# angela000/DQNFlappyBird

Hardware: AMD Instinct MI355X
Metric: env steps/sec (whole node) + DQN grad-steps/sec, 80x80x4 batch=32 (higher is better)
Workload: dtype f32

## Files before the change

dqnflappybird_amd/_lib.py:

```python
import ctypes as C
import os

_HERE = os.path.dirname(os.path.abspath(__file__))
LIB_PATH = os.environ.get("FB_LIB") or os.path.join(_HERE, "libfbdqn.so")
ASSET_BLOB = os.path.join(_HERE, "assets", "sprites.bin")

FB_OK = 0
REPLAY_UNIFORM, REPLAY_PER = 0, 1
RNG_CPYTHON, RNG_PHILOX, RNG_NUMPY = 0, 1, 2
ARCH_PLAIN, ARCH_DUELING, ARCH_C51, ARCH_C51_DUELING = 0, 1, 2, 3
NET_ONLINE, NET_TARGET = 0, 1
ALGO_DQN, ALGO_NATURE, ALGO_DOUBLE, ALGO_PER, ALGO_PG = 0, 1, 2, 3, 4
ALGO_C51, ALGO_C51_DOUBLE = 5, 6
ALGO_C51_PER, ALGO_C51_DOUBLE_PER = 7, 8
C51_MAX_ATOMS = 64
ARCH_QR, ARCH_QR_DUELING = 4, 5
ALGO_QR, ALGO_QR_DOUBLE, ALGO_QR_PER, ALGO_QR_DOUBLE_PER = 9, 10, 11, 12
ALGO_MDQN, ALGO_MDQN_PER = 14, 15
MDQN_DEFAULTS = (0.03, 0.9, -1.0)
ALGO_DOUBLE_PER = 16
ARCH_AC = 6
AC_DEFAULTS = (0.5, 0.01)
ARCH_SAC = 7
SAC_DEFAULTS = (0.2, 0.98, 0.0)
# ... 109 lines not shown
    "fb_qnet_set_iqn_risk": [_vp, _f],
    "fb_qnet_get_iqn": [_vp, _vp, _vp, _vp, _vp, _vp],
    "fb_qnet_set_iqn_munchausen": [_vp, _i, _f, _f, _f],
    "fb_qnet_get_iqn_munchausen": [_vp, _vp, _vp, _vp, _vp],
    "fb_qnet_forward_iqn": [_vp, _i, _vp, _i, _vp, _i, _vp, _vp],
    "fb_iqn_draw_taus": [_i, _i, _u64, _u64, _i, _vp, _vp],
    "fb_qnet_iqn_train_step": [_vp, _i, _i, _vp, _vp, _vp, _vp, _vp, _vp, _vp, _u64, _u64, _d, _vp, _vp, _vp, _vp],
    "fb_iqn_train_from_replay": [_vp, _vp, _i, _i, _vp, _vp, _vp, _vp, _vp, _vp, _u64, _u64, _d, _vp, _vp, _vp, _vp],
    "fb_iqn_step": [_vp, _vp, _vp, _vp, _i, _i, _i, _f, _u64, _u64, _i, _d, _vp],
    "fb_qnet_iqn_per_train_step": [_vp, _i, _i, _vp, _vp, _vp, _vp, _vp, _vp, _vp, _vp, _u64, _u64, _d, _vp, _vp, _vp, _vp, _vp],
    "fb_iqn_per_train_from_replay": [_vp, _vp, _i, _i, _vp, _vp, _vp, _vp, _vp, _vp, _vp, _u64, _u64, _d, _vp, _vp, _vp, _vp, _vp],
    "fb_iqn_per_step": [_vp, _vp, _vp, _vp, _i, _i, _i, _f, _u64, _u64, _i, _d, _vp],
    "fb_qnet_destroy": [_vp],
    "fb_qnet_num_params": [_vp, _vp],
    "fb_qnet_init_params": [_vp, _i, _u64, _vp],
    "fb_qnet_load_params": [_vp, _i, _vp, _vp],
    "fb_qnet_store_params": [_vp, _i, _vp, _vp],
    "fb_qnet_get_adam_state": [_vp] * 4,
    "fb_qnet_set_adam_state": [_vp] * 4,
    "fb_qnet_set_hparams": [_vp, _f, _f, _f, _f],
    "fb_qnet_set_inference_dtype": [_vp, _i],
    "fb_qnet_overflow_count": [_vp, _i, _vp],
    "fb_qnet_split_stats": [_vp, _vp, _vp],
    "fb_vec_step_set_schedule": [_i],
    "fb_qnet_set_train_dtype": [_vp, _i],
    "fb_qnet_forward": [_vp, _i, _vp, _i, _vp, _vp],
    "fb_qnet_act": [_vp, _vp, _i, _f, _u64, _u64, _vp, _vp, _vp],
    "fb_qnet_act_nib": [_vp, _vp, _i, _f, _u64, _u64, _vp, _vp, _vp],
    "fb_qnet_train_step": [_vp, _i, _i] + [_vp] * 6 + [_d] + [_vp] * 5,
    "fb_qnet_apply_adam": [_vp, _vp, _vp],
    "fb_train_steps": [_vp, _vp, _i, _i, _i] + [_vp] * 7 + [_d, _vp],
    "fb_qnet_sync_target": [_vp, _vp],
    "fb_qnet_profile_kernel": [_vp, _i, _i, _i, _i] + [_vp] * 7,
    "fb_dist_probe": [C.c_char_p],
    "fb_dist_unique_id": [C.c_char_p, _vp],
    "fb_dist_create": [C.c_char_p, _i, _i, _vp],
    "fb_dist_destroy": [_vp],
    "fb_dist_set_overlap": [_vp, _i],
    "fb_vec_step_dp": [_vp, _vp, _vp, _vp, _vp, _i, _i, _i, _f, _u64, _u64, _i, _d, _i, _vp],
    "fb_dist_reduce_apply": [_vp, _vp, _vp, _i, _vp],
    "fb_dist_grad_event": [_vp],
    "fb_dist_all_reduce": [_vp, _vp, _i64, _vp],
    "fb_qnet_set_grad_event": [_vp, _vp],
    "fb_qnet_grad_split": [_vp],
    "fb_train_from_replay": [_vp, _vp, _i, _i, _vp, _vp, _vp, _vp, _vp, _d, _vp, _vp, _vp, _vp],
    "fb_profile_ring_kernel": [_vp, _vp, _i, _i, _i, _i] + [_vp] * 6,
    "fb_qnet_kernel_name": [_i],
    "fb_vec_step": [_vp, _vp, _vp, _vp, _i, _i, _i, _f, _u64, _u64, _i, _d, _vp],
    "fb_eval_create": [_i, _vp, _sz, _vp],
    "fb_eval_destroy": [_vp],
    "fb_eval_run": [_vp, _vp, _i, _i, _i64, _f, _u64, _u64, _vp, _vp, _vp, _vp, _vp],
    "fb_eval_stats": [_vp, _vp, _vp],
    "fb_eval_q": [_vp, _vp, _i, _vp, _vp],
}


class StepBuffers(C.Structure):
    _fields_ = [(n, C.c_void_p) for n in ("nib", "actions", "frame_bits", "reward", "terminal", "score", "idx", "s", "s2", "a", "t",
                                           "r", "loss", "flat_grad", "isw", "isw32", "abs_err")]


class AcRolloutBuffers(C.Structure):
    _fields_ = [(n, C.c_void_p) for n in ("nib", "actions", "frame_bits", "reward", "terminal", "score", "value", "logp")] + [("slots", C.c_int)]


_lib = None
# ... 55 lines not shown
```

dqnflappybird_amd/csrc/fb_qnet.hip:

```cpp
#include <math.h>
#include <stdlib.h>
#include "fb_common.h"

#ifndef FK_ABL
#define FK_ABL 0
#endif
#ifndef BW_ABL
#define BW_ABL 0
#endif

namespace {

typedef float f32x16 __attribute__((ext_vector_type(16)));

constexpr int OFF_W1 = 0, OFF_B1 = 8192, OFF_W2 = 8224, OFF_B2 = 40992, OFF_W3 = 41056, OFF_B3 = 77920,
              OFF_WF1 = 77984;
constexpr int CONV_PARAMS = OFF_WF1;
#include "fb_head.h"
#include "fb_sampler.h"
#include "fb_gather.h"
constexpr int MAXTB = 256;


struct Slice { const float *params; const uint8_t *states; int s_off, count; const uint16_t *w1s; int fshift; };
// ... 1831 lines not shown
    if (threadIdx.x >= 256) return;
    const int reg = threadIdx.x >> 6, row = 4 * g + reg, col = r, mr = m0 + row, unit = n0 + col;
    float v = red[reg * 64 + lane];
#pragma unroll
    for (int w = 1; w < 8; w++) v += red[(w * 4 + reg) * 64 + lane];
    const bool live = mr < M;
    const size_t srow = (size_t)s.s_off + (live ? mr : M - 1);
    if (live) a.hf[srow * a.FC + unit] = v;
    if (!a.qpart || FK_ABL == 4) return;
    const float h = fmaxf(v + hb, 0.f);
    const int qs = a.A + 1;
    float *qo = a.qpart + (srow * (size_t)gridDim.y + blockIdx.y) * qs;
#pragma unroll
    for (int c = 0; c <= MAXA; c++) {
        if (c < a.A || (c == a.A && a.dueling)) {
            float x = h * (c == a.A ? hw[MAXA] : hw[c]);
#pragma unroll
            for (int o = 8; o > 0; o >>= 1) x += __shfl_xor(x, o, 16);
            if (col == 0 && live) qo[c] = x;
        }
    }
}

struct Bw1Args {
    int algo, B, FC, A, dueling, stot, n_dx, rb;
    NetOff off;
    const float *params, *pnext, *ptarget;
    const float *hf, *qpart, *h3;
    const uint8_t *act; const float *rew; const uint8_t *term; const float *isw;
    double gamma;
    float *grad, *dh3, *loss, *abs_err, *y_out;
    AdamDev *adam; int tick;
    FbGate gate;
};
constexpr int BW_DX_ROW = 4;
constexpr int BW_DW_ROW = 36;

template <int AT, bool DX, bool MD = false, bool DP = false, bool HU = false>
__device__ __forceinline__ void fc1_bwd2_body(const Bw1Args &L, float *smem, const MdPar M = MdPar{}, const float delta = 0.f) {
    const int tid = threadIdx.x, lane = tid & 63, wave = tid >> 6, B = L.B, FC = L.FC, A = AT == MAXA ? L.A : AT;
    const float *P = L.params;
    float (*dadv)[MAXA] = reinterpret_cast<float (*)[MAXA]>(smem);
    float *dv = smem + MAXTB * MAXA, *lterm = dv + MAXTB, *dadv2 = lterm + MAXTB, *big = dadv2 + 2 * MAXTB;
    const bool lead = blockIdx.x == 0;
    const bool dbl = DP || L.algo == FB_ALGO_DOUBLE;
    const bool row3 = MD || dbl;
    const int qs = A + 1, ntile = FC >> 4;
    constexpr bool dx_role = DX;
    const int mt = dx_role ? blockIdx.x / 50 : 0, t2 = dx_role ? 0 : blockIdx.x - L.n_dx, nt = t2 / 7, kg = t2 - nt * 7;
    const int kt = dx_role ? blockIdx.x - mt * 50 : kg * 8 + wave;
    auto unit_params = [&](int n, float &bias, float (&wq)[AT], float &wv) {
        bias = P[L.off.bf1 + n];
        wv = P[(L.dueling ? L.off.wv : L.off.bf1) + n];
#pragma unroll
        for (int c = 0; c < AT; c++) wq[c] = P[L.off.wq + n * A + (c < A ? c : 0)];
    };
    float pre_hf[32], pre_bias, pre_wq[AT], pre_wv, pre_a[16];
    float4 pre_w[8];
    if constexpr (DX) {
        const int ch = FC < 512 ? FC : 512, n = tid < ch ? tid : 0;
#pragma unroll
        for (int q = 0; q < 32; q++) { const int bq_ = mt * 32 + q; pre_hf[q] = L.hf[(size_t)(bq_ < B ? bq_ : 0) * FC + n]; }
        unit_params(n, pre_bias, pre_wq, pre_wv);
        const int kh = ch / 16, nbeg = wave * (ch / 8) + (lane >> 5) * kh;
        const float *brun = P + OFF_WF1 + (size_t)(kt * 32 + (lane & 31)) * FC + nbeg;
#pragma unroll
        for (int q = 0; q < 8; q++) pre_w[q] = *reinterpret_cast<const float4 *>(brun + (4 * q < kh ? 4 * q : 0));
#pragma unroll
        for (int q = 0; q < 16; q++) pre_a[q] = 0.f;
#pragma unroll
        for (int q = 0; q < 2; q++) { const int mr = mt * 32 + drow(2 * (wave & 7) + q, lane); pre_a[q] = L.h3[(size_t)(mr < B ? mr : 0) * 1600 + kt * 32 + (lane & 31)]; }
    } else {
        const int c = tid & 31;
#pragma unroll
        for (int q = 0; q < 2; q++) { const int b = (tid >> 5) + 16 * q; pre_hf[q] = L.hf[(size_t)(b < B ? b : 0) * FC + nt * 32 + c]; }
#pragma unroll
        for (int q = 2; q < 32; q++) pre_hf[q] = 0.f;
        unit_params(nt * 32 + c, pre_bias, pre_wq, pre_wv);
        const int ktc = kt < 50 ? kt : 0;
#pragma unroll
        for (int t = 0; t < 16; t++) { const int b = 2 * t + (lane >> 5); pre_a[t] = L.h3[(size_t)(b < B ? b : 0) * 1600 + ktc * 32 + (lane & 31)]; }
#pragma unroll
        for (int q = 0; q < 8; q++) pre_w[q] = make_float4(0.f, 0.f, 0.f, 0.f);
// ... 172 lines not shown
                }
            }
            __syncthreads();
            const int kh = ch / 16, nbeg = wave * (ch / 8) + hl * kh;
            const float *arun = dh + i * RS + nbeg;
            float4 xa[8];
#pragma unroll
            for (int q = 0; q < 8; q++) xa[q] = *reinterpret_cast<const float4 *>(arun + (4 * q < kh ? 4 * q : 0));
#pragma unroll
            for (int q = 0; q < 8; q++) { keep(xa[q].x); keep(xa[q].y); keep(xa[q].z); keep(xa[q].w); }
#pragma unroll
            for (int q = 0; q < 8; q++) {
                if (4 * q < kh && BW_ABL != 3) {
                    const float4 x = xa[q], w = pre_w[q];
                    const bool rb = L.rb;
                    acc = mfma(rbf(x.x, rb), rbf(w.x, rb), acc); acc = mfma(rbf(x.y, rb), rbf(w.y, rb), acc);
                    acc = mfma(rbf(x.z, rb), rbf(w.z, rb), acc); acc = mfma(rbf(x.w, rb), rbf(w.w, rb), acc);
                }
            }
        }
        reduce_rows<8>(acc, red, wave, lane, mt * 32, B, [&](float v, int r, int mr) {
            const size_t o = (size_t)mr * 1600 + kt * 32 + jj;
            L.dh3[o] = BW_ABL == 4 ? v : (((r & 1) ? pre_a[1] : pre_a[0]) > 0.f ? v : 0.f);
        });
        return;
    }
    if (BW_ABL == 5) return;
    float *dh = big, *hh = big + MAXTB * BW_DW_ROW;
    {
        const int c = tid & 31;
#pragma unroll
        for (int q = 0; q < 2; q++) {
            const int b = (tid >> 5) + 16 * q;
            if (b < B) { float hv; dh[b * BW_DW_ROW + c] = dhf_of(b, pre_hf[q], pre_bias, pre_wq, pre_wv, hv); hh[b * BW_DW_ROW + c] = hv; }
        }
        for (int b = (tid >> 5) + 32; b < B; b += 16) {
            float hv;
            dh[b * BW_DW_ROW + c] = dhf_of(b, L.hf[(size_t)b * FC + nt * 32 + c], pre_bias, pre_wq, pre_wv, hv);
            hh[b * BW_DW_ROW + c] = hv;
        }
    }
    __syncthreads();
    if (kt < 50) {
        f32x16 acc = {0};
#pragma unroll
        for (int t = 0; t < 16; t++) {
            const int b = 2 * t + hl;
            const float w = dh[(b < B ? b : 0) * BW_DW_ROW + jj];
            acc = mfma(b < B ? rbf(pre_a[t], L.rb) : 0.f, b < B ? rbf(w, L.rb) : 0.f, acc);
        }
#pragma unroll 4
        for (int t = 16; t < (B + 1) / 2; t++) {
            const int b = 2 * t + hl, bc = b < B ? b : 0;
            const float x = L.h3[(size_t)bc * 1600 + kt * 32 + i], w = dh[bc * BW_DW_ROW + jj];
            acc = mfma(b < B ? rbf(x, L.rb) : 0.f, b < B ? rbf(w, L.rb) : 0.f, acc);
        }
#pragma unroll
        for (int r = 0; r < 16; r++) L.grad[OFF_WF1 + (size_t)(kt * 32 + drow(r, lane)) * FC + nt * 32 + jj] = acc[r];
    }
    if (kg != 0) return;
    float *part = hh + MAXTB * BW_DW_ROW;
    {
        const int c = tid & 31, pt = tid >> 5;
        float gw[AT], gv = 0.f, gb = 0.f;
#pragma unroll
        for (int q = 0; q < AT; q++) gw[q] = 0.f;
        for (int b = pt; b < B; b += 16) {
            const float h = hh[b * BW_DW_ROW + c];
#pragma unroll
            for (int q = 0; q < AT; q++) if (q < A) gw[q] = fmaf(h, dadv[b][q], gw[q]);
            gv = fmaf(h, dv[b], gv);
            gb += dh[b * BW_DW_ROW + c];
// ... 403 lines not shown
    auto ld = [&](int ks) {
        const int b0 = 16 * (k0 + ks) + 8 * hl;
        float a[8], bb[8];
#pragma unroll
        for (int j = 0; j < 8; j++) {
            const bool ok = b0 + j < B;
            const size_t bc = ok ? b0 + j : 0;
            const float x = pa[bc * 1600], y = pb[bc * FC];
            a[j] = ok ? x : 0.f; bb[j] = ok ? y : 0.f;
        }
        return FragF{make_float4(a[0], a[1], a[2], a[3]), make_float4(a[4], a[5], a[6], a[7]), make_float4(bb[0], bb[1], bb[2], bb[3]),
                     make_float4(bb[4], bb[5], bb[6], bb[7])};
    };
    const Pow2 G = pow2_scale(wave_max(gm));
    if constexpr (KW > 0) {
        FragF f[KW];
#pragma unroll
        for (int q = 0; q < KW; q++) f[q] = ld(q);
#pragma unroll
        for (int q = 0; q < KW; q++) mma_frag<NS, false>(f[q], acc, acl, G.s, bad);
    } else {
        for (int q = 0; q < per; q++) mma_frag<NS, false>(ld(q), acc, acl, G.s, bad);
    }
    if constexpr (NS == 3) {
#pragma unroll
        for (int q = 0; q < 16; q++) acc[q] = fmaf(acl[q], F16_LO_UNSCALE, acc[q]) * G.inv;
        note_overflow(bad, ovf);
    }
    reduce_rows<8>(acc, red, wave, lane, 0, 32, [&](float v, int, int row32) {
        grad[OFF_WF1 + (size_t)(it * 32 + row32) * FC + nt * 32 + r] = v;
    });
}

__device__ __forceinline__ void adam4(float4 &P, float4 &Mv, float4 &V, const float4 Gv, float alpha, float omb1, float omb2, float eps) {
#define FB_ADAM1(c)                                  \
    Mv.c += (Gv.c - Mv.c) * omb1;                    \
    V.c += (Gv.c * Gv.c - V.c) * omb2;               \
    P.c -= (Mv.c * alpha) / (sqrtf(V.c) + eps);
    FB_ADAM1(x) FB_ADAM1(y) FB_ADAM1(z) FB_ADAM1(w)
#undef FB_ADAM1
}

struct AdamSpan { float *p, *m, *v; const float *g; const AdamDev *ad; int q0, q1; };
__device__ __forceinline__ void adam_span_body(int blk, int nblk, const AdamSpan a) {
    const float alpha = a.ad->alpha, omb1 = 1.f - a.ad->b1, omb2 = 1.f - a.ad->b2, eps = a.ad->eps;
    for (int q = a.q0 + blk * (int)blockDim.x + (int)threadIdx.x; q < a.q1; q += nblk * (int)blockDim.x) {
        float4 P = reinterpret_cast<float4 *>(a.p)[q], Mv = reinterpret_cast<float4 *>(a.m)[q], V = reinterpret_cast<float4 *>(a.v)[q];
        adam4(P, Mv, V, reinterpret_cast<const float4 *>(a.g)[q], alpha, omb1, omb2, eps);
        reinterpret_cast<float4 *>(a.p)[q] = P; reinterpret_cast<float4 *>(a.m)[q] = Mv; reinterpret_cast<float4 *>(a.v)[q] = V;
    }
}

constexpr int DW1_IMG_W = 104, DW1_IMG_H = 84, DW1_IMG = DW1_IMG_H * DW1_IMG_W * 4;
constexpr int DW1_STEPS = 30;

template <int NSP> struct Dw1Lds { static constexpr int U4 = DW1_IMG / 16 + (DW1_STEPS / NSP) * 2 * 64 + 64 + 4; };

struct Dw1Ring { const unsigned long long *bits, *fo; };
template <int NSP, bool RING = false>
__device__ __forceinline__ void conv1_dw2_body(int blk, const uint8_t *__restrict__ states, const float *__restrict__ dp1,
                                               const uint8_t *__restrict__ amax, float *__restrict__ slabs, size_t slab_stride, uint4 *pool,
                                               Dw1Ring ring = Dw1Ring{nullptr, nullptr}) {
    constexpr int SW = DW1_STEPS / NSP, PU = (SW + 7) / 8;
    uint4 *img4 = pool, *bfr = pool + DW1_IMG / 16;
    float (*bsum)[32] = reinterpret_cast<float (*)[32]>(bfr + SW * 2 * 64);
    float *sx = reinterpret_cast<float *>(bfr + SW * 2 * 64 + 64);
    const int b = blk / NSP, part = blk - b * NSP, s0 = part * SW;
    const int tid = threadIdx.x, lane = tid & 63, wave = tid >> 6, hl = lane >> 5, c = lane & 31;
    uint8_t *img = reinterpret_cast<uint8_t *>(img4);
    float dv[PU][4];
    int am[PU][4];
#pragma unroll
    for (int u = 0; u < PU; u++) {
        const int ls = wave + 8 * u, g = 2 * (s0 + ls) + hl, oy = g / 3, ox0 = (g - 3 * oy) * 8;
#pragma unroll
        for (int q = 0; q < 4; q++) {
            const int px = (ox0 >> 1) + q;
            const bool ok = ls < SW && px < 10;
            const uint32_t po = ((uint32_t)b * 100u + (uint32_t)(ok ? (oy >> 1) * 10 + px : 0)) * 32u + (uint32_t)c;
            dv[u][q] = dp1[po]; am[u][q] = amax[po];
        }
    }
// ... 281 lines not shown
    Ops cur = fetch(0);
#pragma unroll
    for (int ls = 0; ls < SW; ls++) {
        Ops nxt = cur;
        if (ls + 1 < SW) nxt = fetch(ls + 1);
        uint4 A;
        {
            const f32x2 p0 = {(float)cur.x[0], (float)cur.x[1]}, p1 = {(float)cur.x[2], (float)cur.x[3]};
            const f32x2 p2 = {(float)cur.x[4], (float)cur.x[5]}, p3 = {(float)cur.x[6], (float)cur.x[7]};
            A.x = __builtin_bit_cast(uint32_t, __builtin_convertvector(p0, f16x2)); A.y = __builtin_bit_cast(uint32_t, __builtin_convertvector(p1, f16x2));
            A.z = __builtin_bit_cast(uint32_t, __builtin_convertvector(p2, f16x2)); A.w = __builtin_bit_cast(uint32_t, __builtin_convertvector(p3, f16x2));
        }
        acc = mfma_h(A, cur.bh, acc);
        acl = mfma_h(A, cur.bl, acl);
        cur = nxt;
    }
    float *o = slabs + (size_t)blk * slab_stride;
#pragma unroll
    for (int r = 0; r < 16; r++) o[OFF_W1 + (ky * 32 + drow(r, lane)) * 32 + c] = fmaf(acl[r], F16_LO_UNSCALE, acc[r]) * S1.inv;
    if (wave == 0 && hl == 0) {
        float sum = bsum[0][c];
#pragma unroll
        for (int w = 1; w < 8; w++) sum += bsum[w][c];
        o[OFF_B1 + c] = sum;
    }
}

#ifndef CBW_ABL
#define CBW_ABL 0
#endif
template <int NS, bool RING>
__global__ __launch_bounds__(512) void conv_bw_kernel(BxArgs bx, int B, float *__restrict__ slabs, size_t slab_stride, float *__restrict__ slabs1,
                                                      size_t stride1, const uint8_t *__restrict__ states, const uint8_t *__restrict__ amax, Dw1Ring ring,
                                                      int n_adam, AdamSpan span, FbSampleRider rider, int rb, FbGate gate) {
    __shared__ uint4 pool[BwLds<NS>::U4];
    if (fb_gate_workgroup(gate)) return;
    static_assert(BwLds<NS>::U4 * 16 >= FB_SAMPLE_LDS_WORDS * 4, "the sampler rider borrows the pool");
    uint4 *aux = pool + BwLds<NS>::CH;
    float *dp1s = reinterpret_cast<float *>(aux + BW_AUX_U4);
    const int rid = rider.k ? 1 : 0, bid = (int)blockIdx.x - rid, tid = threadIdx.x;
    if (bid < 0) {
        uint32_t *sw = reinterpret_cast<uint32_t *>(pool);
        if (tid < 64) sample_cpython_body(rider.ctx, rider.k, rider.setsize, rider.out, sw, reinterpret_cast<int *>(sw + 624));
        return;
    }
    if (bid < 2 * B) {
        if (CBW_ABL == 5 || CBW_ABL == 6 || CBW_ABL == 7 || CBW_ABL == 8 || CBW_ABL == 11) return;
        const int b = bid >> 1, part = bid & 1;
        const Bw1Pre pre = bw1_request<RING>(b, part, states, amax, ring);
        for (int i = tid; i < BW1_IMG_U4; i += 512) aux[i] = make_uint4(0u, 0u, 0u, 0u);
        conv32_bx_body<NS, 1>(bx, b, pool, dp1s);
        bw1_put(pre, part, aux);
        __syncthreads();
        if (CBW_ABL == 1 || CBW_ABL == 10) { if (dp1s[tid] == 12345.f) slabs1[0] = 1.f; return; }
        bw1_main(bid, part, pre, dp1s, aux, pool + (BwLds<NS>::CH - 2048 - 4), slabs1, stride1);
        return;
    }
    if (bid < (2 + BW_NW2) * B) {
        if (CBW_ABL == 6 || CBW_ABL == 7 || CBW_ABL == 9 || CBW_ABL == 10) return;
        const int b = (bid - 2 * B) / BW_NW2, sub = (bid - 2 * B) - b * BW_NW2;
        float *p1s = reinterpret_cast<float *>(aux), *dys = p1s + 3200;
        const float4 *src = reinterpret_cast<const float4 *>(bx.p1 + (size_t)b * 3200);
        const float4 xa = src[tid], xb = src[tid < 288 ? 512 + tid : 0];
        reinterpret_cast<float4 *>(p1s)[tid] = xa;
        if (tid < 288) reinterpret_cast<float4 *>(p1s)[512 + tid] = xb;
        conv32_bx_body<NS, 2>(bx, b, pool, dys);
        __syncthreads();
        float *o = slabs + (size_t)b * slab_stride;
        if (CBW_ABL == 2 || CBW_ABL == 11) { if (dys[tid] == 12345.f) o[0] = 1.f; return; }
        dw_sample_tiles<2>(p1s, dys, o, rb, sub, BW_NW2);
        if (sub == BW_NW2 - 1) dw_sample_bias(dys, o + OFF_B2);
        return;
    }
    if (bid < BW_WGS * B) {
        if (CBW_ABL == 3 || CBW_ABL == 6 || CBW_ABL == 8 || CBW_ABL == 9 || CBW_ABL == 10 || CBW_ABL == 11) return;
        const int b = (bid - (2 + BW_NW2) * B) / BW_NW3, sub = (bid - (2 + BW_NW2) * B) - b * BW_NW3;
        float *dys = reinterpret_cast<float *>(aux), *xs = dys + 1600;
        const int q = tid < 400 ? tid : 0;
        const float4 d = reinterpret_cast<const float4 *>(bx.dh3 + (size_t)b * 1600)[q], x = reinterpret_cast<const float4 *>(bx.h2 + (size_t)b * 1600)[q];
        if (tid < 400) { reinterpret_cast<float4 *>(dys)[tid] = d; reinterpret_cast<float4 *>(xs)[tid] = x; }
        __syncthreads();
        float *o = slabs + (size_t)b * slab_stride;
        dw_sample_tiles<3>(xs, dys, o, rb, sub, BW_NW3);
        if (sub == BW_NW3 - 1) dw_sample_bias(dys, o + OFF_B3);
        return;
    }
    if (CBW_ABL == 4) return;
    adam_span_body(bid - BW_WGS * B, n_adam, span);
}

template <int NS> struct DwgLds {
    static constexpr int NPL = NS == 3 ? 2 : 1, PLH = 25 * 32 * 16;
    static constexpr int U4 = 2 * NPL * PLH / 8 + 64 + 128 + 2048 + 4;
};

template <int NS, int LAYER>
__device__ __forceinline__ void conv_dwg_body(int blk, const float *__restrict__ x, const float *__restrict__ dy, float *__restrict__ slabs,
                                              size_t slab_stride, uint4 *pool, unsigned *ovf) {
    constexpr int NPL = DwgLds<NS>::NPL, PLH = DwgLds<NS>::PLH, ZERO = 2 * NPL * PLH;
    uint16_t *X = reinterpret_cast<uint16_t *>(pool), *DY = X + NPL * PLH;
    float *part = reinterpret_cast<float *>(pool + 2 * NPL * PLH / 8 + 64);
    float *red = part + 512;
    float *sx = red + 8192;
    const int tid = threadIdx.x, lane = tid & 63, wave = tid >> 6, hl = lane >> 5, r = lane & 31;
    const int cot = blk & 1, mid = LAYER == 3 ? (blk >> 1) & 1 : (blk >> 1) & 3, g = LAYER == 3 ? blk >> 2 : blk >> 3;
    const int py = mid >> 1, px = mid & 1;
    float xa[13], xb[13], ya[13], yb[13];
#pragma unroll
    for (int q = 0; q < 13; q++) {
        const int w = wave + 8 * q, wc = w < 100 ? w : 0, pos = wc % 25, bp = wc / 25 + 4 * hl;
        const size_t s0 = (size_t)g * 16 + 2 * bp;
        size_t xo;
        if (LAYER == 3) xo = (s0 * 25 + pos) * 64 + mid * 32 + r;
        else { const int qy = pos / 5, qx = pos - qy * 5; xo = (s0 * 100 + (py + 2 * qy) * 10 + px + 2 * qx) * 32 + r; }
        const size_t yo = (s0 * 25 + pos) * 64 + cot * 32 + r;
        xa[q] = x[xo]; xb[q] = x[xo + (LAYER == 3 ? 1600 : 3200)];
        ya[q] = dy[yo]; yb[q] = dy[yo + 1600];
    }
    if (tid < 64) pool[2 * NPL * PLH / 8 + tid] = make_uint4(0u, 0u, 0u, 0u);
    Pow2 SY = {1.f, 1.f};
// ... 1101 lines not shown
        if (dp) L.algo = FB_ALGO_PER;
        const dim3 grid(FC / 16);
        if (dp || hu) fb_qnet_launch_loss_head_x(dp, hu, md, grid.x, c.st, &L, &h->md, h->huber);
        else if (md) hipLaunchKernelGGL(loss_head_md_kernel, grid, dim3(256), 0, c.st, L, h->md);
        else hipLaunchKernelGGL(loss_head_kernel, grid, dim3(256), 0, c.st, L);
        return;
    }
    const bool pw = is_per_algo(p.algo);
    auto dist = [&](auto &L) {
        shared(L); transition(L); L.off = h->hoff;
        L.p_on = head_base(h, h->params[0]); L.p_next = head_base(h, p.sl.s[1].params);
        L.p_tgt = head_base(h, p.ns > 2 ? p.sl.s[2].params : p.sl.s[1].params);
        L.dl = h->c51_dl; L.xs = h->c51_xs; L.lterm = h->c51_lt;
        L.isw = pw ? p.isw : nullptr; L.abs_err = pw ? p.abs_err : nullptr;
    };
    with_actions(h->A, [&](auto a) { with_bool(pw, [&](auto w) {
        if (is_qr(h)) {
            QRLossArgs L;
            dist(L);
            L.algo = is_double_qr(p.algo) ? FB_ALGO_QR_DOUBLE : FB_ALGO_QR; L.N = h->sup.N; L.kappa = h->kappa;
            hipLaunchKernelGGL((qr_loss_kernel<decltype(a)::value, decltype(w)::value>), dim3((B + 3) / 4), dim3(256), 0, c.st, L);
        } else {
            C51LossArgs L;
            dist(L);
            L.algo = is_double_c51(p.algo) ? FB_ALGO_C51_DOUBLE : FB_ALGO_C51; L.sup = h->sup;
            hipLaunchKernelGGL((c51_loss_kernel<decltype(a)::value, decltype(w)::value>), dim3((B + 3) / 4), dim3(256), 0, c.st, L);
        }
    }); });
    const C51GradArgs gA{B, FC, h->A, h->sup.N, h->off, h->c51_dl, h->c51_xs, h->c51_lt, h->dhf, p.a, p.G, p.loss, h->gmax, h->adam, p.tick};
    if (is_c51d(h)) hipLaunchKernelGGL(c51d_grad_kernel, dim3(FC / 16), dim3(256), 0, c.st, gA);
    else hipLaunchKernelGGL(c51_grad_kernel, dim3(FC / 16), dim3(256), 0, c.st, gA);
}

static void fc1_backward(fb_qnet *h, const Plan &p, const PlanCtx &c) {
    const int B = p.B, FC = h->FC;
    if (!c.big && !c.c51 && !c.ac) {
        const int ndx1 = ((B + 31) / 32) * 50;
        Bw1Args L;
        L.algo = p.algo; L.B = B; L.FC = FC; L.A = h->A; L.dueling = h->arch == FB_ARCH_DUELING; L.stot = c.stot; L.n_dx = ndx1; L.off = h->off;
        L.params = h->params[0]; L.pnext = p.sl.s[1].params; L.ptarget = p.ns > 2 ? p.sl.s[2].params : p.sl.s[1].params;
        L.hf = h->hf; L.qpart = h->qpart; L.h3 = h->h3; L.act = p.a; L.rew = p.r; L.term = p.t; L.isw = p.isw; L.gamma = p.gamma;
        L.grad = p.G; L.dh3 = h->dh3; L.loss = p.loss; L.abs_err = p.abs_err; L.y_out = p.y;
        L.adam = h->adam; L.tick = p.tick; L.rb = h->nsplit_train == 1;
        L.gate = p.split && c.only < 0 ? FbGate{&p.split->f->trunk_done, p.split->seq, &p.split->f->timeouts[2]} : FbGate{nullptr, 0, nullptr};
        const dim3 grid(ndx1 + (FC / 32) * 7 + (L.gate.flag ? 1 : 0));
        const bool dp = p.algo == FB_ALGO_DOUBLE_PER, hu = h->huber > 0.f, md = is_mdqn_algo(p.algo);
        if (md) L.algo = p.algo == FB_ALGO_MDQN_PER ? FB_ALGO_PER : FB_ALGO_NATURE;
        if (dp) L.algo = FB_ALGO_PER;
        if (dp || hu) fb_qnet_launch_fc1_bwd2_x(dp, hu, md, grid.x, c.st, &L, &h->md, h->huber);
        else if (md) hipLaunchKernelGGL(fc1_bwd2_md_kernel, grid, dim3(512), 0, c.st, L, h->md);
        else hipLaunchKernelGGL(fc1_bwd2_kernel, grid, dim3(512), 0, c.st, L);
        return;
    }
    const int ndx = ((B + 31) / 32) * 50, ntile = ndx + 50 * (FC / 32);
    const bool std_shape = FC == 512 && B == 256;
    with_nsp(h->nsplit_train, [&](auto ns) { with_bool(std_shape, [&](auto s) {
        hipLaunchKernelGGL((fc1_bwd_big_kernel<decltype(ns)::value, decltype(s)::value ? 4 : 0, decltype(s)::value ? 2 : 0>), dim3(ntile), dim3(512), 0, c.st,
                           ndx, h->params[0], h->h3, h->dhf, h->dh3, p.G, B, FC, (const float *)h->gmax, &h->adam->ovf);
    }); });
}

struct SlabCounts { int z1, z3; };
static SlabCounts conv_backward(fb_qnet *h, const Plan &p, const PlanCtx &c, int span0, int span1) {
    const int B = p.B, FC = h->FC, rbt = h->nsplit_train == 1;
    int z3 = min((B * 25 + 255) / 256, h->zmax);
    const size_t ss = CONV_PARAMS;
    const AdamSpan span{master(h, 0), h->adam_m, h->adam_v, p.G, h->adam, span0, span1};
    const FbGate gate_fc1 = p.split && c.only < 0 ? FbGate{&p.split->f->fc1_done, p.split->seq, &p.split->f->timeouts[3]} : FbGate{nullptr, 0, nullptr};
    const FbSampleRider srider = p.sample_rider ? *p.sample_rider : FbSampleRider{};
    const bool fold1 = 2 * B > h->zmax;
    const int fold = (2 * B + h->zmax - 1) / h->zmax;
    const int z1 = fold1 ? (2 * B + fold - 1) / fold : 2 * B;
    const int n_adam5 = (span1 - span0 + 511) / 512;
    const BxArgs bx{h->dh3, h->h2, h->p1, h->dh2, h->dp1, h->wsp[0] + wsp_w3t(FC), h->wsp[0] + wsp_w2t(FC)};
    const Dw1Ring dr{p.ring ? p.ring->c.bits : nullptr, h->ring_fo};
    float *s1 = fold1 ? h->slabs1 : h->slabs;
    const size_t st1 = fold1 ? (size_t)CONV1_PARAMS : ss;
    const bool dwg = c.big && B % 16 == 0;
    const int zt3 = dwg ? 0 : z3, zt2 = zt3;
    const bool bw = !c.big && B <= h->zmax;
    if (bw) {
        z3 = B;
        const dim3 g(BW_WGS * B + n_adam5 + (srider.k ? 1 : 0) + (gate_fc1.flag ? 1 : 0));
        if (runs(c, K_CONV3_BWD)) with_nsp(h->nsplit_train, [&](auto ns) { with_bool(p.ring != nullptr, [&](auto r) {
            hipLaunchKernelGGL((conv_bw_kernel<decltype(ns)::value, decltype(r)::value>), g, dim3(512), 0, c.st,
                               bx, B, h->slabs, ss, s1, st1, p.s, (const uint8_t *)h->amax, dr, n_adam5, span, srider, rbt, gate_fc1);
        }); });
    } else {
        const dim3 g3(B + 38 * zt3 + n_adam5 + (srider.k ? 1 : 0)), g2(34 * zt2 + 2 * B + (gate_fc1.flag ? 1 : 0));
        if (runs(c, K_CONV3_BWD)) with_nsp(h->nsplit_train, [&](auto ns) {
            hipLaunchKernelGGL(conv_bx_kernel<decltype(ns)::value>, g3, dim3(512), 0, c.st, bx, B, zt3, h->slabs, ss, n_adam5, span, srider, rbt);
        });
        if (dwg) {
            z3 = B / 16;
            const int n3 = z3 * 4, n2 = z3 * 8;
            if (runs(c, K_CONV2_BWD)) with_nsp(h->nsplit_train, [&](auto ns) {
                hipLaunchKernelGGL(conv_dwg_kernel<decltype(ns)::value>, dim3(n3 + n2), dim3(512), 0, c.st, n3, h->h2, h->dh3, h->p1, h->dh2, h->slabs, ss, &h->adam->ovf);
            });
        }
        if (runs(c, K_CONV2_BWD)) with_bool(p.ring != nullptr, [&](auto r) {
            hipLaunchKernelGGL((conv_dw21_kernel<2, decltype(r)::value>), g2, dim3(512), 0, c.st,
                               zt2, B, h->p1, h->dh2, p.s, h->dp1, h->amax, h->slabs, ss, s1, st1, rbt, dr, gate_fc1);
        });
    }
    if (fold1 && runs(c, K_CONV2_BWD)) hipLaunchKernelGGL(slab_fold_kernel, dim3((CONV1_PARAMS + 255) / 256, z1), dim3(256), 0, c.st, h->slabs1, 2 * B, fold, h->slabs, ss);
    return SlabCounts{z1, z3};
}

static void reduce_or_adam(fb_qnet *h, const Plan &p, const PlanCtx &c, SlabCounts z, int span1) {
    if (p.split && c.only < 0) h->split_adam_pending = !p.apply_adam;
    if (!p.apply_adam && runs(c, K_SLAB)) hipLaunchKernelGGL(slab_reduce_kernel, dim3((CONV_PARAMS / 4 + 255) / 256), dim3(256), 0, c.st, h->slabs, (size_t)CONV_PARAMS, z.z1, z.z3, z.z3, p.G);
    if (c.only < 0) noisy_sgrad(h, p.G, c.st);
    if (p.apply_adam && runs(c, K_ADAM)) {
        AdamFused af;
        af.p = master(h, 0); af.m = h->adam_m; af.v = h->adam_v; af.g = p.G; af.n = h->ntot; af.ad = h->adam;
        af.slabs = h->slabs; af.slab_stride = CONV_PARAMS; af.z1 = z.z1; af.z2 = af.z3 = z.z3;
        af.w1s = h->w1s[0]; af.wsp = h->wsp[0]; af.FC = h->FC; af.tail0 = span1;
        const long long nrest4 = OFF_W2 / 4 + (OFF_W3 - OFF_B2) / 4 + (OFF_WF1 - OFF_B3) / 4 + (h->ntot / 4 - span1);
        af.lanes = 4;
// ... 843 lines not shown
                                          const uint8_t *t, const float *isw, const float *tau, const float *tau_next, uint64_t seed, uint64_t step,
                                          double gamma, float *loss, float *abs_err, float *q_target, float *flat_grad, void *stream) {
    FB_REQUIRE(h && s && a && r && s2 && t && loss, "fb_qnet_iqn_per_train_step: NULL argument");
    FB_REQUIRE(isw && abs_err, "fb_qnet_iqn_per_train_step: the prioritized step needs the importance weights (isw) and abs_err");
    return iqn_train("fb_qnet_iqn_per_train_step", h, double_q, B, s, a, r, s2, t, nullptr, isw, tau, tau_next, seed, step, gamma, loss, abs_err, q_target,
                     flat_grad, stream);
}

int fb_qnet_iqn_train_ring(fb_qnet_t h, int double_q, int B, const FbRingSrc *ring, const float *isw, const float *tau, const float *tau_next,
                           uint64_t seed, uint64_t step, double gamma, float *loss, float *abs_err, float *q_target, float *flat_grad, void *stream,
                           const char *who) {
    FB_REQUIRE(h && ring && ring->idx && ring->a && ring->r && ring->t && loss && !isw == !abs_err, "%s: NULL argument", who);
    return iqn_train(who, h, double_q, B, nullptr, ring->a, ring->r, nullptr, ring->t, ring, isw, tau, tau_next, seed, step, gamma, loss, abs_err, q_target,
                     flat_grad, stream);
}

extern "C" int fb_qnet_profile_kernel(fb_qnet_t h, int kernel, int reps, int algo, int B, const uint8_t *s, const uint8_t *a,
                                      const float *r, const uint8_t *s2, const uint8_t *t, float *loss, void *stream) {
    FB_REQUIRE(kernel >= 0 && kernel < K_COUNT && reps >= 1, "fb_qnet_profile_kernel: bad kernel id / reps");
    Plan p;
    int rc = FB_OK;
    if (algo < 0) {
        FB_REQUIRE(h && s && B >= 1 && B <= 3 * h->max_batch && kernel <= K_HEAD, "fb_qnet_profile_kernel: bad forward request");
        p = forward_plan(h, 0, s, B);
        p.nib = algo == -2;
    } else rc = train_plan(h, algo, B, s, a, r, s2, t, nullptr, 0.99, loss, nullptr, nullptr, nullptr, &p);
    if (rc != FB_OK) return rc;
    p.tick = false;
    for (int n = 0; n < 2; n++) resplit_now(h, n, fb_stream(stream));
    for (int i = 0; i < reps; i++) { rc = run_plan(h, p, kernel, fb_stream(stream)); if (rc != FB_OK) return rc; }
    return FB_OK;
}

extern "C" const char *fb_qnet_kernel_name(int kernel) {
    static const char *names[K_COUNT] = {"conv1_pool_kernel", "conv23_t_kernel", "(conv3: in conv23_t)", "fc1_fk_kernel", "head_kernel",
                                         "(loss: in fc1_bwd2)", "fc1_bwd2_kernel", "conv_bw_kernel", "(conv2 / conv1 dW: in conv_bw)",
                                         "(conv1 dW: in conv_bw)", "slab_reduce_kernel", "adam_fused_kernel"};
    return kernel >= 0 && kernel < K_COUNT ? names[kernel] : "";
}
#endif
```

include/fbdqn.h:

```cpp
#ifndef FBDQN_H
#define FBDQN_H
#include <stddef.h>
#include <stdint.h>

#ifdef __cplusplus
extern "C" {
#endif

#define FB_OK 0
#define FB_ERR_INVALID (-1)
#define FB_ERR_HIP (-2)
#define FB_ERR_NOMEM (-3)
#define FB_ERR_STATE (-4)

const char *fb_last_error(void);
int fb_version(void);
int fb_device_count(void);
int fb_debug_abort_backtrace(void);

typedef struct fb_env *fb_env_t;

#define FB_ENV_STATE_INTS 16

int fb_env_create(int n_envs, uint64_t seed, uint32_t flags, const void *sprite_blob, size_t blob_bytes,
// ... 203 lines not shown
int fb_qnet_create_iqn_dueling(int fc_width, int n_actions, int n_tau, int n_tau_next, int n_tau_act, float kappa, int max_batch, fb_qnet_t *out);
int fb_qnet_set_iqn_munchausen(fb_qnet_t h, int on, float temp, float alpha, float clip_lo);
int fb_qnet_get_iqn_munchausen(fb_qnet_t h, int *on_host, float *temp_host, float *alpha_host, float *clip_lo_host);

int fb_qnet_create(int arch, int fc_width, int n_actions, int max_batch, fb_qnet_t *out);
int fb_qnet_destroy(fb_qnet_t h);
int fb_qnet_num_params(fb_qnet_t h, int64_t *n_host);
int fb_qnet_init_params(fb_qnet_t h, int which, uint64_t seed, void *stream);
int fb_qnet_load_params(fb_qnet_t h, int which, const float *flat , void *stream);
int fb_qnet_store_params(fb_qnet_t h, int which, float *flat , void *stream);
int fb_qnet_get_adam_state(fb_qnet_t h, float *m, float *v, float *beta_pows_host);
int fb_qnet_set_adam_state(fb_qnet_t h, const float *m, const float *v, const float *beta_pows_host);
int fb_qnet_set_hparams(fb_qnet_t h, float lr, float beta1, float beta2, float eps);
#define FB_DTYPE_F32 0
#define FB_DTYPE_BF16 1
int fb_qnet_set_inference_dtype(fb_qnet_t h, int dtype);
int fb_qnet_overflow_count(fb_qnet_t h, int reset, int64_t *count_host);
int fb_qnet_set_train_dtype(fb_qnet_t h, int dtype);
int fb_qnet_forward(fb_qnet_t h, int which, const uint8_t *states, int batch, float *q, void *stream);
int fb_qnet_act(fb_qnet_t h, const uint8_t *states, int n, float epsilon, uint64_t seed, uint64_t step,
                uint8_t *actions, float *q, void *stream);
int fb_qnet_act_nib(fb_qnet_t h, const uint8_t *nib_states, int n, float epsilon, uint64_t seed, uint64_t step,
                    uint8_t *actions, float *q, void *stream);
int fb_qnet_train_step(fb_qnet_t h, int algo, int batch, const uint8_t *s, const uint8_t *a, const float *r,
                       const uint8_t *s2, const uint8_t *t, const float *isw, double gamma, float *loss,
                       float *abs_err, float *q_target, float *flat_grad, void *stream);
int fb_qnet_apply_adam(fb_qnet_t h, const float *flat_grad, void *stream);
int fb_qnet_set_grad_event(fb_qnet_t h, void *event);
int64_t fb_qnet_grad_split(fb_qnet_t h);
int fb_qnet_sync_target(fb_qnet_t h, void *stream);
int fb_qnet_profile_kernel(fb_qnet_t h, int kernel, int reps, int algo, int batch, const uint8_t *s, const uint8_t *a,
                           const float *r, const uint8_t *s2, const uint8_t *t, float *loss, void *stream);
const char *fb_qnet_kernel_name(int kernel);

typedef struct {
    uint8_t *nib;
    uint8_t *actions;
    uint64_t *frame_bits;
    float *reward; uint8_t *terminal; int32_t *score;
    int64_t *idx;
    uint8_t *s, *s2, *a, *t; float *r;
    float *loss;
    float *flat_grad;
    double *isw; float *isw32; float *abs_err;
} fb_step_buffers;
int fb_qnet_split_stats(fb_qnet_t net, int64_t *steps_host, int64_t *clean_host);
int fb_vec_step_set_schedule(int split);
int fb_vec_step(fb_env_t env, fb_replay_t replay, fb_qnet_t net, const fb_step_buffers *b, int n_envs, int algo, int batch,
                float epsilon, uint64_t seed, uint64_t step, int train, double gamma, void *stream);
int fb_sac_step(fb_env_t env, fb_replay_t replay, fb_qnet_t net, const fb_step_buffers *b, int n_envs, int batch, uint64_t seed, uint64_t step,
                int train, double gamma, float rho, void *stream);
int fb_sac_per_step(fb_env_t env, fb_replay_t replay, fb_qnet_t net, const fb_step_buffers *b, int n_envs, int batch, uint64_t seed, uint64_t step,
                    int train, double gamma, float rho, void *stream);
int fb_iqn_step(fb_env_t env, fb_replay_t replay, fb_qnet_t net, const fb_step_buffers *b, int n_envs, int double_q, int batch, float epsilon,
                uint64_t seed, uint64_t step, int train, double gamma, void *stream);
int fb_iqn_per_step(fb_env_t env, fb_replay_t replay, fb_qnet_t net, const fb_step_buffers *b, int n_envs, int double_q, int batch, float epsilon,
                    uint64_t seed, uint64_t step, int train, double gamma, void *stream);

int fb_train_from_replay(fb_replay_t replay, fb_qnet_t net, int algo, int batch, const int64_t *idx, const float *isw, uint8_t *a, float *r,
                         uint8_t *t, double gamma, float *loss, float *abs_err, float *flat_grad, void *stream);
int fb_profile_ring_kernel(fb_replay_t replay, fb_qnet_t net, int kernel, int reps, int algo, int batch, const int64_t *idx, uint8_t *a,
                           float *r, uint8_t *t, float *loss, void *stream);

typedef struct fb_dist *fb_dist_t;
int fb_dist_probe(const char *librccl_path);
int fb_dist_unique_id(const char *librccl_path, uint8_t *id128 );
// ... 27 lines not shown
```

Measured before the change: 11.32 million.

## Move fc1 weight-gradient into conv_bw Adam span, fusing dW with Adam update

The fc1 backward kernel now publishes its dhf activations-gradient to a global buffer and launches only one block per output tile instead of seven. The fc1 weight gradient (h3^T·dhf via MFMA) is then computed inside conv_bw_kernel's Adam workgroups, where each tile applies the Adam update directly without writing the gradient to memory first. This removes the fc1 dW grid from fc1_bwd2, removes a gradient write and read, and overlaps the work with conv backward. The cost is an extra global write of dhf, and the dW work now sits on a different kernel's critical path. A helper to copy the fc1 operands is also exported.

```diff
diff --git a/dqnflappybird_amd/_lib.py b/dqnflappybird_amd/_lib.py
--- a/dqnflappybird_amd/_lib.py
+++ b/dqnflappybird_amd/_lib.py
@@ -165,6 +165,7 @@
     "fb_train_steps": [_vp, _vp, _i, _i, _i] + [_vp] * 7 + [_d, _vp],
     "fb_qnet_sync_target": [_vp, _vp],
     "fb_qnet_profile_kernel": [_vp, _i, _i, _i, _i] + [_vp] * 7,
+    "fb_qnet_copy_fc1_operands": [_vp, _i, _vp, _vp, _vp],
     "fb_dist_probe": [C.c_char_p],
     "fb_dist_unique_id": [C.c_char_p, _vp],
     "fb_dist_create": [C.c_char_p, _i, _i, _vp],
diff --git a/dqnflappybird_amd/csrc/fb_qnet.hip b/dqnflappybird_amd/csrc/fb_qnet.hip
--- a/dqnflappybird_amd/csrc/fb_qnet.hip
+++ b/dqnflappybird_amd/csrc/fb_qnet.hip
@@ -1887,6 +1887,7 @@
     float *grad, *dh3, *loss, *abs_err, *y_out;
     AdamDev *adam; int tick;
     FbGate gate;
+    float *dhf;
 };
 constexpr int BW_DX_ROW = 4;
 constexpr int BW_DW_ROW = 36;
@@ -1902,8 +1903,9 @@
     const bool row3 = MD || dbl;
     const int qs = A + 1, ntile = FC >> 4;
     constexpr bool dx_role = DX;
-    const int mt = dx_role ? blockIdx.x / 50 : 0, t2 = dx_role ? 0 : blockIdx.x - L.n_dx, nt = t2 / 7, kg = t2 - nt * 7;
-    const int kt = dx_role ? blockIdx.x - mt * 50 : kg * 8 + wave;
+    const bool pub = !dx_role && L.dhf != nullptr;
+    const int mt = dx_role ? blockIdx.x / 50 : 0, t2 = dx_role ? 0 : blockIdx.x - L.n_dx, nt = pub ? t2 : t2 / 7, kg = pub ? 0 : t2 - nt * 7;
+    const int kt = dx_role ? blockIdx.x - mt * 50 : pub ? 50 : kg * 8 + wave;
     auto unit_params = [&](int n, float &bias, float (&wq)[AT], float &wv) {
         bias = P[L.off.bf1 + n];
         wv = P[(L.dueling ? L.off.wv : L.off.bf1) + n];
@@ -2142,12 +2144,18 @@
 #pragma unroll
         for (int q = 0; q < 2; q++) {
             const int b = (tid >> 5) + 16 * q;
-            if (b < B) { float hv; dh[b * BW_DW_ROW + c] = dhf_of(b, pre_hf[q], pre_bias, pre_wq, pre_wv, hv); hh[b * BW_DW_ROW + c] = hv; }
+            if (b < B) {
+                float hv;
+                const float d = dhf_of(b, pre_hf[q], pre_bias, pre_wq, pre_wv, hv);
+                dh[b * BW_DW_ROW + c] = d; hh[b * BW_DW_ROW + c] = hv;
+                if (pub) L.dhf[(size_t)b * FC + nt * 32 + c] = d;
+            }
         }
         for (int b = (tid >> 5) + 32; b < B; b += 16) {
             float hv;
-            dh[b * BW_DW_ROW + c] = dhf_of(b, L.hf[(size_t)b * FC + nt * 32 + c], pre_bias, pre_wq, pre_wv, hv);
-            hh[b * BW_DW_ROW + c] = hv;
+            const float d = dhf_of(b, L.hf[(size_t)b * FC + nt * 32 + c], pre_bias, pre_wq, pre_wv, hv);
+            dh[b * BW_DW_ROW + c] = d; hh[b * BW_DW_ROW + c] = hv;
+            if (pub) L.dhf[(size_t)b * FC + nt * 32 + c] = d;
         }
     }
     __syncthreads();
@@ -2617,13 +2625,14 @@
     });
 }
 
+__device__ __forceinline__ void adam1(float &P, float &Mv, float &V, const float G, float alpha, float omb1, float omb2, float eps) {
+    Mv += (G - Mv) * omb1;
+    V += (G * G - V) * omb2;
+    P -= (Mv * alpha) / (sqrtf(V) + eps);
+}
 __device__ __forceinline__ void adam4(float4 &P, float4 &Mv, float4 &V, const float4 Gv, float alpha, float omb1, float omb2, float eps) {
-#define FB_ADAM1(c)                                  \
-    Mv.c += (Gv.c - Mv.c) * omb1;                    \
-    V.c += (Gv.c * Gv.c - V.c) * omb2;               \
-    P.c -= (Mv.c * alpha) / (sqrtf(V.c) + eps);
-    FB_ADAM1(x) FB_ADAM1(y) FB_ADAM1(z) FB_ADAM1(w)
-#undef FB_ADAM1
+    adam1(P.x, Mv.x, V.x, Gv.x, alpha, omb1, omb2, eps); adam1(P.y, Mv.y, V.y, Gv.y, alpha, omb1, omb2, eps);
+    adam1(P.z, Mv.z, V.z, Gv.z, alpha, omb1, omb2, eps); adam1(P.w, Mv.w, V.w, Gv.w, alpha, omb1, omb2, eps);
 }
 
 struct AdamSpan { float *p, *m, *v; const float *g; const AdamDev *ad; int q0, q1; };
@@ -2633,6 +2642,51 @@
         float4 P = reinterpret_cast<float4 *>(a.p)[q], Mv = reinterpret_cast<float4 *>(a.m)[q], V = reinterpret_cast<float4 *>(a.v)[q];
         adam4(P, Mv, V, reinterpret_cast<const float4 *>(a.g)[q], alpha, omb1, omb2, eps);
         reinterpret_cast<float4 *>(a.p)[q] = P; reinterpret_cast<float4 *>(a.m)[q] = Mv; reinterpret_cast<float4 *>(a.v)[q] = V;
+    }
+}
+struct DwSpan { const float *h3, *dhf; int FC; };
+__device__ __forceinline__ void fc1_dw_adam_body(int blk, const AdamSpan a, const DwSpan d, int B, bool rb) {
+    const int lane = threadIdx.x & 63, wave = threadIdx.x >> 6, hl = lane >> 5, jj = lane & 31;
+    const int FC = d.FC, ntn = FC >> 5, tile = blk * 8 + wave;
+    if (tile >= 50 * ntn) return;
+    const int kt = tile / ntn, nt = tile - kt * ntn;
+    const float alpha = a.ad->alpha, omb1 = 1.f - a.ad->b1, omb2 = 1.f - a.ad->b2, eps = a.ad->eps;
+    auto at = [](const float *base, int off) { return reinterpret_cast<const float *>(reinterpret_cast<const char *>(base) + (unsigned)off); };
+    auto to = [](float *base, int off) { return reinterpret_cast<float *>(reinterpret_cast<char *>(base) + (unsigned)off); };
+    const int a0 = 4 * (kt * 32 + jj), w0 = 4 * (nt * 32 + jj);
+    float pre_a[16], pre_w[16];
+#pragma unroll
+    for (int t = 0; t < 16; t++) {
+        const int b = 2 * t + hl, bc = b < B ? b : 0;
+        pre_a[t] = *at(d.h3, a0 + bc * 6400); pre_w[t] = *at(d.dhf, w0 + bc * 4 * FC);
+    }
+    __builtin_amdgcn_sched_barrier(0);
+    float P[16], Mv[16], V[16];
+    const int o0 = 4 * (OFF_WF1 + (kt * 32 + 4 * hl) * FC + nt * 32 + jj);
+#pragma unroll
+    for (int r = 0; r < 16; r++) { const int o = o0 + 4 * ((r & 3) + 8 * (r >> 2)) * FC; P[r] = *at(a.p, o); Mv[r] = *at(a.m, o); V[r] = *at(a.v, o); }
+#pragma unroll
+    for (int t = 0; t < 16; t++) { keep(pre_a[t]); keep(pre_w[t]); }
+    f32x16 acc = {0};
+#pragma unroll
+    for (int t = 0; t < 16; t++) {
+        const int b = 2 * t + hl;
+        acc = mfma(b < B ? rbf(pre_a[t], rb) : 0.f, b < B ? rbf(pre_w[t], rb) : 0.f, acc);
+    }
+#pragma unroll 4
+    for (int t = 16; t < (B + 1) / 2; t++) {
+        const int b = 2 * t + hl, bc = b < B ? b : 0;
+        const float x = *at(d.h3, a0 + bc * 6400), w = *at(d.dhf, w0 + bc * 4 * FC);
+        acc = mfma(b < B ? rbf(x, rb) : 0.f, b < B ? rbf(w, rb) : 0.f, acc);
+    }
+    int o1 = o0;
+    keep(o1);
+#pragma unroll
+    for (int r = 0; r < 16; r++) {
+        if ((r & 3) == 0) __builtin_amdgcn_sched_barrier(0);
+        const int o = o1 + 4 * ((r & 3) + 8 * (r >> 2)) * FC;
+        adam1(P[r], Mv[r], V[r], acc[r], alpha, omb1, omb2, eps);
+        *to(a.p, o) = P[r]; *to(a.m, o) = Mv[r]; *to(a.v, o) = V[r];
     }
 }
 
@@ -2980,17 +3034,22 @@
 template <int NS, bool RING>
 __global__ __launch_bounds__(512) void conv_bw_kernel(BxArgs bx, int B, float *__restrict__ slabs, size_t slab_stride, float *__restrict__ slabs1,
                                                       size_t stride1, const uint8_t *__restrict__ states, const uint8_t *__restrict__ amax, Dw1Ring ring,
-                                                      int n_adam, AdamSpan span, FbSampleRider rider, int rb, FbGate gate) {
+                                                      int n_adam, AdamSpan span, DwSpan dw, FbSampleRider rider, int rb, FbGate gate) {
     __shared__ uint4 pool[BwLds<NS>::U4];
     if (fb_gate_workgroup(gate)) return;
     static_assert(BwLds<NS>::U4 * 16 >= FB_SAMPLE_LDS_WORDS * 4, "the sampler rider borrows the pool");
     uint4 *aux = pool + BwLds<NS>::CH;
     float *dp1s = reinterpret_cast<float *>(aux + BW_AUX_U4);
-    const int rid = rider.k ? 1 : 0, bid = (int)blockIdx.x - rid, tid = threadIdx.x;
+    const int rid = rider.k ? 1 : 0, tid = threadIdx.x;
+    int bid = (int)blockIdx.x - rid;
     if (bid < 0) {
         uint32_t *sw = reinterpret_cast<uint32_t *>(pool);
         if (tid < 64) sample_cpython_body(rider.ctx, rider.k, rider.setsize, rider.out, sw, reinterpret_cast<int *>(sw + 624));
         return;
+    }
+    if (dw.dhf) {
+        if (bid >= 2 * B && bid < 2 * B + n_adam) { if (CBW_ABL != 4) fc1_dw_adam_body(bid - 2 * B, span, dw, B, rb != 0); return; }
+        if (bid >= 2 * B + n_adam) bid -= n_adam;
     }
     if (bid < 2 * B) {
         if (CBW_ABL == 5 || CBW_ABL == 6 || CBW_ABL == 7 || CBW_ABL == 8 || CBW_ABL == 11) return;
@@ -3034,6 +3093,7 @@
         return;
     }
     if (CBW_ABL == 4) return;
+    if (dw.dhf) return;
     adam_span_body(bid - BW_WGS * B, n_adam, span);
 }
 
@@ -4201,10 +4261,15 @@
     else hipLaunchKernelGGL(c51_grad_kernel, dim3(FC / 16), dim3(256), 0, c.st, gA);
 }
 
+static bool dw_in_span(const fb_qnet *h, const Plan &p, const PlanCtx &c) {
+    return p.apply_adam && !c.big && !c.c51 && !c.ac && p.B <= h->zmax && !h->noisy;
+}
+
 static void fc1_backward(fb_qnet *h, const Plan &p, const PlanCtx &c) {
     const int B = p.B, FC = h->FC;
     if (!c.big && !c.c51 && !c.ac) {
         const int ndx1 = ((B + 31) / 32) * 50;
+        const bool span_dw = dw_in_span(h, p, c);
         Bw1Args L;
         L.algo = p.algo; L.B = B; L.FC = FC; L.A = h->A; L.dueling = h->arch == FB_ARCH_DUELING; L.stot = c.stot; L.n_dx = ndx1; L.off = h->off;
         L.params = h->params[0]; L.pnext = p.sl.s[1].params; L.ptarget = p.ns > 2 ? p.sl.s[2].params : p.sl.s[1].params;
@@ -4212,7 +4277,8 @@
         L.grad = p.G; L.dh3 = h->dh3; L.loss = p.loss; L.abs_err = p.abs_err; L.y_out = p.y;
         L.adam = h->adam; L.tick = p.tick; L.rb = h->nsplit_train == 1;
         L.gate = p.split && c.only < 0 ? FbGate{&p.split->f->trunk_done, p.split->seq, &p.split->f->timeouts[2]} : FbGate{nullptr, 0, nullptr};
-        const dim3 grid(ndx1 + (FC / 32) * 7 + (L.gate.flag ? 1 : 0));
+        L.dhf = span_dw ? h->dhf : nullptr;
+        const dim3 grid(ndx1 + (FC / 32) * (span_dw ? 1 : 7) + (L.gate.flag ? 1 : 0));
         const bool dp = p.algo == FB_ALGO_DOUBLE_PER, hu = h->huber > 0.f, md = is_mdqn_algo(p.algo);
         if (md) L.algo = p.algo == FB_ALGO_MDQN_PER ? FB_ALGO_PER : FB_ALGO_NATURE;
         if (dp) L.algo = FB_ALGO_PER;
@@ -4250,10 +4316,13 @@
     const bool bw = !c.big && B <= h->zmax;
     if (bw) {
         z3 = B;
-        const dim3 g(BW_WGS * B + n_adam5 + (srider.k ? 1 : 0) + (gate_fc1.flag ? 1 : 0));
+        const bool span_dw = dw_in_span(h, p, c);
+        const DwSpan dw{h->h3, span_dw ? h->dhf : nullptr, FC};
+        const int n_span = span_dw ? (50 * (FC / 32) + 7) / 8 : n_adam5;
+        const dim3 g(BW_WGS * B + n_span + (srider.k ? 1 : 0) + (gate_fc1.flag ? 1 : 0));
         if (runs(c, K_CONV3_BWD)) with_nsp(h->nsplit_train, [&](auto ns) { with_bool(p.ring != nullptr, [&](auto r) {
             hipLaunchKernelGGL((conv_bw_kernel<decltype(ns)::value, decltype(r)::value>), g, dim3(512), 0, c.st,
-                               bx, B, h->slabs, ss, s1, st1, p.s, (const uint8_t *)h->amax, dr, n_adam5, span, srider, rbt, gate_fc1);
+                               bx, B, h->slabs, ss, s1, st1, p.s, (const uint8_t *)h->amax, dr, n_span, span, dw, srider, rbt, gate_fc1);
         }); });
     } else {
         const dim3 g3(B + 38 * zt3 + n_adam5 + (srider.k ? 1 : 0)), g2(34 * zt2 + 2 * B + (gate_fc1.flag ? 1 : 0));
@@ -5163,6 +5232,13 @@
     return FB_OK;
 }
 
+extern "C" int fb_qnet_copy_fc1_operands(fb_qnet_t h, int batch, float *h3, float *dhf, void *stream) {
+    FB_REQUIRE(h && batch >= 1 && batch <= h->max_batch, "fb_qnet_copy_fc1_operands: batch must be in 1..max_batch");
+    if (h3) FB_CHECK_HIP(hipMemcpyAsync(h3, h->h3, sizeof(float) * (size_t)batch * 1600, hipMemcpyDeviceToDevice, fb_stream(stream)));
+    if (dhf) FB_CHECK_HIP(hipMemcpyAsync(dhf, h->dhf, sizeof(float) * (size_t)batch * h->FC, hipMemcpyDeviceToDevice, fb_stream(stream)));
+    return FB_OK;
+}
+
 extern "C" const char *fb_qnet_kernel_name(int kernel) {
     static const char *names[K_COUNT] = {"conv1_pool_kernel", "conv23_t_kernel", "(conv3: in conv23_t)", "fc1_fk_kernel", "head_kernel",
                                          "(loss: in fc1_bwd2)", "fc1_bwd2_kernel", "conv_bw_kernel", "(conv2 / conv1 dW: in conv_bw)",
diff --git a/include/fbdqn.h b/include/fbdqn.h
--- a/include/fbdqn.h
+++ b/include/fbdqn.h
@@ -259,6 +259,7 @@
 int fb_qnet_profile_kernel(fb_qnet_t h, int kernel, int reps, int algo, int batch, const uint8_t *s, const uint8_t *a,
                            const float *r, const uint8_t *s2, const uint8_t *t, float *loss, void *stream);
 const char *fb_qnet_kernel_name(int kernel);
+int fb_qnet_copy_fc1_operands(fb_qnet_t h, int batch, float *h3, float *dhf, void *stream);
 
 typedef struct {
     uint8_t *nib;
```

Measured after the change: 11.36 million, median of 5. About the same (+0.4%).
